# robertknight/rten

Measured on NVIDIA H100. Metric: resnet50_fp32_inferences_per_sec, higher is better.
Workload: dtype f32(tf32 mma, explicit opt-in)

## Files before the change

rten_b200/csrc/umma_gemm.cu:

```cuda
#include <cuda.h>
#include <cuda_runtime.h>

#include <algorithm>
#include <array>
#include <cmath>
#include <vector>
#include <cmath>
#include <cstdint>
#include <cstdio>
#include <cstdlib>

#include "math.cuh"
#include "ptx.cuh"
#include "rowops.h"
#include "umma_gemm.h"
#include "umma_kernel.cuh"

namespace rtb {

typedef CUresult (*EncodeTiledFn)(CUtensorMap*, CUtensorMapDataType, cuuint32_t, void*, const cuuint64_t*,
                                  const cuuint64_t*, const cuuint32_t*, const cuuint32_t*, CUtensorMapInterleave,
                                  CUtensorMapSwizzle, CUtensorMapL2promotion, CUtensorMapFloatOOBfill);

static EncodeTiledFn get_encode(rten_ctx* ctx) {
// ... 399 lines not shown
    if (!encode_map(ctx, &m.a, L.a, q.esize, L.kind == 0, q.abox, q.aes)) return RTEN_ERR_UNSUPPORTED_VALUE;
    if (!encode_map(ctx, &m.b, L.b, q.esize, L.kind == 0, bbox, bes)) return RTEN_ERR_UNSUPPORTED_VALUE;
    m.d = m.r = m.a2 = m.a_proj = m.b_proj = m.a2_proj = m.w2 = m.z = m.a;
    p.x3_cb = L.x3_cb;
    if (L.x3_cb && !encode_map(ctx, &m.a2, L.a_lo, q.esize, true, q.abox, q.aes)) return RTEN_ERR_UNSUPPORTED_VALUE;
    if (p.kb_proj) {
        p.x3_cb_proj = L.proj.x3_cb;
        if (!encode_map(ctx, &m.a_proj, L.proj.a, 4, true, q.pbox, q.pes) ||
            !encode_map(ctx, &m.b_proj, L.proj.b, 4, true, bbox, bes) ||
            (L.proj.x3_cb && !encode_map(ctx, &m.a2_proj, L.proj.a_lo, 4, true, q.pbox, q.pes)))
            return RTEN_ERR_UNSUPPORTED_VALUE;
    }
    if (p.tma_store && !encode_map(ctx, &m.d, q.od, 4, true, q.dbox, des)) {
        p.tma_store = 0;
        p.res_tma = 0;
        m.d = m.a;
    }
    if (p.res_tma && !encode_map(ctx, &m.r, q.ord, 4, true, q.dbox, des)) {
        p.res_tma = 0;
        m.r = m.a;
    }
    const Epi epi = pick_epilogue(L, p.tma_store, p.res_tma, p.splitk);
    if (epi == Epi::Generic && (L.kind == 1 || L.epi.act > 1)) p.res_tma = 0;
    if (q.chain_bytes) {
        const GemmLaunch::Chain& c = L.chain;
        const uint32_t wbox[4] = {32, (uint32_t)c.N2, 1, 1}, zbox[4] = {32, q.dbox[1], q.dbox[2], q.dbox[3]};
        if (epi != Epi::PlainF32 || (L.epi.r && !p.res_tma) || !encode_map(ctx, &m.w2, c.w, 4, true, wbox, des) ||
            !encode_map(ctx, &m.z, c.z, 4, true, zbox, des))
            return RTEN_ERR_UNSUPPORTED_VALUE;
        p.chain_n2 = c.N2;
        p.chain_passes = (L.N + p.bn - 1) / p.bn;
        p.chain_act = c.act;
        p.chain_bias = c.bias;
    }

    if (verbose)
        fprintf(stderr, "[umma_gemm] kind=%d conv=%d M=%d N=%d K=%d kb=%d kb_proj=%d tiles_m=%d bn=%d splitk=%d units=%d stages=%d tma_store=%d res_tma=%d nbuf=%d box=%dx%dx%d epi=%s%s\n",
                L.kind, L.conv, L.M, L.N, L.K, p.k_blocks, p.kb_proj, p.tiles_m, p.bn, p.splitk, p.units_total, p.stages,
                p.tma_store, p.res_tma, p.nbuf, p.tw, p.th, p.tb, epi_name(epi),
                p.chain_n2 == 64 ? " chain=64" : p.chain_n2 == 128 ? " chain=128" : "");
    if ((is_wide(p.bn) || p.kb_proj || L.epi.bias2) && !is_plain_f32(epi)) return RTEN_ERR_UNSUPPORTED_VALUE;
    const size_t smem_bytes = (size_t)p.stages * p.stage_bytes + q.chain_bytes +
                              (is_wide(p.bn) ? WIDE_SMEM_FIXED_BYTES : ps.n_stg * STG_BYTES + SMEM_FIXED_BYTES);
    using Kernel = void (*)(TmaMaps, KParams);
    static const Kernel narrow[2][7] = {
        {umma_gemm_kernel<0, Epi::Generic>, umma_gemm_kernel<0, Epi::Fast>, umma_gemm_kernel<0, Epi::FastGelu>,
         umma_gemm_kernel<0, Epi::PlainF32>, umma_gemm_kernel<0, Epi::PlainF32Gelu>, nullptr, nullptr},
        {umma_gemm_kernel<1, Epi::Generic>, umma_gemm_kernel<1, Epi::Fast>, umma_gemm_kernel<1, Epi::FastGelu>, nullptr,
         nullptr, umma_gemm_kernel<1, Epi::PlainI8>, umma_gemm_kernel<1, Epi::PlainI8Gelu>}};
    const Kernel kern = !is_wide(p.bn)              ? narrow[L.kind][(int)epi]
                        : p.chain_n2 == 64         ? umma_wide_kernel<Epi::PlainF32, 64>
                        : p.chain_n2 == 128        ? umma_wide_kernel<Epi::PlainF32, 128>
                        : epi == Epi::PlainF32Gelu ? umma_wide_kernel<Epi::PlainF32Gelu>
                                                   : umma_wide_kernel<Epi::PlainF32>;

    const int threads = is_wide(p.bn) ? WIDE_THREADS : NUM_THREADS;
    return launch(ctx, "umma_gemm launch", kern, {std::min(p.units_total, ctx->num_sms), threads, smem_bytes, 227 * 1024, true}, m, p);
}

static std::vector<long long> tune_key(const GemmLaunch& L, const Prepared& q) {
    const EpilogueDesc& e = L.epi;
    std::vector<long long> k = {L.kind, L.conv, L.M, L.N, L.K, L.z0, L.z1, q.tma_store, q.res_tma, e.act, e.bias_kind,
                                e.r != nullptr, (e.za != nullptr || e.za8 != nullptr), e.zb != nullptr, e.scale != nullptr,
                                L.a.strides[1], L.b.strides[1], L.x3_cb};
    if (L.conv) {
        const ConvGeom& g = L.g;
        for (long long v : {g.B, g.H, g.W, g.C, g.OH, g.OW, g.kh, g.kw, g.sy, g.sx, g.dy, g.dx, g.pt, g.pl}) k.push_back(v);
    }
    if (L.proj.C > 0) {
        const GemmLaunch::Projection& pr = L.proj;
        for (int64_t v : {(int64_t)-1, (int64_t)pr.C, (int64_t)pr.stride, (int64_t)pr.x3_cb, pr.a.dims[1], pr.a.dims[2],
                          pr.a.strides[1], pr.a.strides[2], pr.a.strides[3], pr.b.strides[1]})
            k.push_back(v);
    }
    return k;
}

static Plan plan_from_array(const std::array<int, 3>& a) {
    Plan pl;
    pl.bn = a[0];
    pl.splitk = a[1];
    pl.nbuf = a[2];
    return pl;
}

static rten_status launch_tf32x3(rten_ctx* ctx, const GemmLaunch& L0) {
    GemmLaunch L = L0;
    long long d0 = 0, d0p = 0;
    auto split = [&](const OperandDesc& src, OperandDesc& dst, int role, void* into) -> rten_status {
        const long long planes = role == 2 ? 1 : 3;
        long long dims[4], strides[4], n = planes * d0p;
        for (int i = 0; i < 4; i++) {
            dims[i] = (i > 0 && src.strides[i] == 0) ? 1 : src.dims[i];
            strides[i] = src.strides[i];
        }
        for (int i = 1; i < 4; i++) n *= dims[i];
        void* buf = into;
        if (!buf) RTB_TRY(temp_alloc(ctx, (size_t)n * 4, &buf));
        RTB_TRY(launch_tf32x3_split(ctx, (const float*)src.base, (float*)buf, dims, strides, d0p, role));
        dst = src;
        dst.base = buf;
        dst.dims[0] = planes * d0p;
        long long st = planes * d0p;
        for (int i = 1; i < 4; i++) {
            dst.strides[i] = (src.strides[i] == 0 && src.dims[i] > 1) ? 0 : st;
            st *= dims[i];
        }
        return RTEN_OK;
    };
    auto split_source = [&](const OperandDesc& a0, const OperandDesc& b0, void** slot, const void* a_lo_base,
                            OperandDesc& a, OperandDesc& b, OperandDesc& a_lo, int& x3_cb) -> rten_status {
        d0 = a0.dims[0];
        d0p = (d0 + 3) / 4 * 4;
        if (b0.dims[0] != d0) return RTEN_ERR_UNSUPPORTED_VALUE;
        if (slot && !getenv("RTEN_B200_X3_NO_CACHE")) {
            if (!*slot && !ctx->capturing) {
                long long n = 3 * d0p;
                for (int i = 1; i < 4; i++) n *= (b0.strides[i] == 0 ? 1 : b0.dims[i]);
                void* buf = nullptr;
                if (cudaMalloc(&buf, (size_t)n * 4) != cudaSuccess) return fail(ctx, RTEN_ERR_CUDA, "cudaMalloc failed for the 3xTF32 copy of a prepacked operand");
                OperandDesc tmp;
                const rten_status st = split(b0, tmp, 1, buf);
                if (st != RTEN_OK) {
                    cudaFree(buf);
                    return st;
                }
                *slot = buf;
            }
        }
        if (slot && *slot && !getenv("RTEN_B200_X3_NO_CACHE")) {
            b = b0;
            b.base = *slot;
            b.dims[0] = 3 * d0p;
            long long st = 3 * d0p;
            for (int i = 1; i < 4; i++) {
                const long long di = b0.strides[i] == 0 ? 1 : b0.dims[i];
                b.strides[i] = (b0.strides[i] == 0 && b0.dims[i] > 1) ? 0 : st;
                st *= di;
            }
        } else {
            RTB_TRY(split(b0, b, 1, nullptr));
        }
        const bool two_plane = d0 % 32 == 0 && tma_compatible(a0, 4, 4) && !getenv("RTEN_B200_X3_THREE_PLANES");
        if (two_plane && a_lo_base) {
            a_lo = a0;
            a_lo.base = a_lo_base;
            x3_cb = (int)(d0 / 32);
        } else if (two_plane) {
            RTB_TRY(split(a0, a_lo, 2, nullptr));
            x3_cb = (int)(d0 / 32);
        } else {
            RTB_TRY(split(a0, a, 0, nullptr));
        }
        return RTEN_OK;
    };
    RTB_TRY(split_source(L0.a, L0.b, L0.b_x3_slot, L0.a_lo_base, L.a, L.b, L.a_lo, L.x3_cb));
    if (L.conv)
        L.g.C = (int)(3 * d0p);
    L.K = L.conv ? (int)(L0.K / d0 * 3 * d0p) : (int)(3 * d0p);
    L.b_x3_slot = nullptr;
    L.a_lo_base = nullptr;
    if (L0.proj.C > 0) {
        RTB_TRY(split_source(L0.proj.a, L0.proj.b, L0.proj.b_x3_slot, nullptr, L.proj.a, L.proj.b, L.proj.a_lo, L.proj.x3_cb));
        L.proj.C = (int)(3 * d0p);
        L.proj.b_x3_slot = nullptr;
    }
    const int saved = ctx->f32_mode;
    ctx->f32_mode = RTEN_F32_TF32;
    const rten_status st = launch_umma_gemm(ctx, L);
    ctx->f32_mode = saved;
    return st;
}

rten_status launch_umma_gemm(rten_ctx* ctx, const GemmLaunch& L) {
    if (L.chain.N2 > 0) {
        if (L.kind != 0 || ctx->f32_mode != RTEN_F32_TF32 || L.x3_cb || getenv("RTEN_B200_NO_CHAIN"))
            return RTEN_ERR_UNSUPPORTED_VALUE;
        Prepared q;
        RTB_TRY(prepare_launch(ctx, L, q));
        Plan pl;
        pl.bn = 128;
        pl.nbuf = 2;
        return launch_plan(ctx, L, q, pl, getenv("RTEN_B200_VERBOSE") != nullptr);
    }
    if (L.kind == 0 && ctx->f32_mode == RTEN_F32_TF32X3) return launch_tf32x3(ctx, L);
    if (L.conv && L.kind == 0 && L.g.kh * L.g.kw > 1 && !L.x3_cb && !L.proj.C) {
        const rten_status hs = launch_umma_halo_conv(ctx, L);
        if (hs != RTEN_ERR_UNSUPPORTED_VALUE) return hs;
    }
    Prepared q;
    RTB_TRY(prepare_launch(ctx, L, q));
    const bool verbose = getenv("RTEN_B200_VERBOSE") != nullptr;
    const bool forced = getenv("RTEN_B200_FORCE_BN") || getenv("RTEN_B200_FORCE_SPLITK");
    if (!forced && !ctx->tune_cache.empty()) {
        auto hit = ctx->tune_cache.find(tune_key(L, q));
        if (hit != ctx->tune_cache.end()) {
            PlanShape ps;
            if (hit->second[0] < 0) {
                const rten_status hs = launch_umma_halo_conv(ctx, L, hit->second[1], hit->second[2]);
                if (hs != RTEN_ERR_UNSUPPORTED_VALUE) return hs;
            } else
            if (plan_shape(q, plan_from_array(hit->second), ps)) return launch_plan(ctx, L, q, plan_from_array(hit->second), verbose);
            if (verbose) fprintf(stderr, "[umma_gemm] recorded plan no longer valid for this problem: re-planning\n");
            ctx->tune_cache.erase(hit);
        }
    }
    std::vector<std::pair<double, Plan>> cands;
    enumerate_plans(q, ctx->num_sms, cands);
    if (cands.empty()) return RTEN_ERR_UNSUPPORTED_VALUE;
    Plan plan = cands[0].second;

    if (forced) {
        const char* fb = getenv("RTEN_B200_FORCE_BN");
        const char* fs = getenv("RTEN_B200_FORCE_SPLITK");
        bool found = false;
        for (const auto& c : cands) {
            const Plan& x = c.second;
            if (fb && x.bn != atoi(fb)) continue;
            if (fs && x.splitk != atoi(fs)) continue;
            plan = x;
            found = true;
            break;
        }
        if (!found) {
            ctx->forced_misses++;
            if (verbose) fprintf(stderr, "[umma_gemm] no valid plan matches the forced fields: using the model's choice\n");
            if (getenv("RTEN_B200_FORCE_STRICT"))
                return fail(ctx, RTEN_ERR_INVALID_VALUE, "no launch plan matches the forced RTEN_B200_FORCE_* fields");
        } else {
            ctx->forced_hits++;
        }
    } else if (ctx->autotune || !ctx->tune_cache.empty()) {
        const std::vector<long long> key = tune_key(L, q);
        auto it = ctx->tune_cache.find(key);
        PlanShape ps_hit;
        if (it != ctx->tune_cache.end() && it->second[0] < 0) {
            const rten_status hs = launch_umma_halo_conv(ctx, L, it->second[1], it->second[2]);
            if (hs != RTEN_ERR_UNSUPPORTED_VALUE) return hs;
            ctx->tune_cache.erase(it);
        } else if (it != ctx->tune_cache.end() && plan_shape(q, plan_from_array(it->second), ps_hit)) {
            plan = plan_from_array(it->second);
        } else if (ctx->autotune) {
            cudaStreamCaptureStatus cs = cudaStreamCaptureStatusNone;
            cudaStreamIsCapturing(ctx->stream, &cs);
            const bool safe = !ctx->capturing && cs == cudaStreamCaptureStatusNone &&
                              (L.epi.r == nullptr || (const void*)L.epi.r != (const void*)L.epi.d);
            if (safe) {
                cudaEvent_t e0, e1;
                cudaEventCreate(&e0);
                cudaEventCreate(&e1);
                const size_t ncand = std::min<size_t>(cands.size(), 24);
                size_t ws_max = 0;
                for (size_t i = 0; i < ncand; i++) {
                    PlanShape ps;
                    if (plan_shape(q, cands[i].second, ps)) ws_max = std::max(ws_max, splitk_ws_bytes(ps, cands[i].second));
                }
                void* ws = nullptr;
                if (ws_max) {
                    RTB_TRY(ensure_splitk_counters(ctx));
                    RTB_TRY(temp_alloc(ctx, ws_max, &ws));
                    cudaStreamSynchronize(ctx->stream);
                }
                double best_ms = 1e30;
                int reps = 4;
                std::vector<std::pair<double, size_t>> timed;
                auto time_plan = [&](const Plan& x, int n) -> double {
                    if (launch_plan(ctx, L, q, x, false, ws) != RTEN_OK) return -1.0;
                    cudaEventRecord(e0, ctx->stream);
                    bool ok = true;
                    for (int r = 0; r < n && ok; r++) ok = launch_plan(ctx, L, q, x, false, ws) == RTEN_OK;
                    cudaEventRecord(e1, ctx->stream);
                    if (cudaEventSynchronize(e1) != cudaSuccess || !ok) return -1.0;
                    float t = 0.f;
                    cudaEventElapsedTime(&t, e0, e1);
                    return (double)t / n;
                };
                for (size_t i = 0; i < ncand; i++) {
                    const Plan& x = cands[i].second;
                    double ms = time_plan(x, reps);
                    if (ms < 0) continue;
                    timed.emplace_back(ms, i);
                    if (verbose)
                        fprintf(stderr, "[autotune] bn=%d splitk=%d nbuf=%d model=%.0f -> %.2f us\n", x.bn, x.splitk, x.nbuf,
                                cands[i].first, ms * 1e3);
                    if (ms < best_ms) {
                        best_ms = ms;
                        plan = x;
                    }
                    reps = std::max(4, std::min(32, (int)(0.15 / std::max(best_ms, 1e-3))));
                }
                std::sort(timed.begin(), timed.end());
                best_ms = 1e30;
                for (size_t k = 0; k < std::min<size_t>(3, timed.size()); k++) {
                    const Plan& x = cands[timed[k].second].second;
                    const double again = time_plan(x, 2 * reps);
                    const double ms = again < 0 ? timed[k].first : again;
                    if (ms < best_ms) {
                        best_ms = ms;
                        plan = x;
                    }
                }
                int halo_bn = 0, halo_T = 0;
                if (L.conv && L.kind == 0 && L.g.kh * L.g.kw > 1 && !L.x3_cb && !L.proj.C && !getenv("RTEN_B200_NO_HALO")) {
                    for (int hbn : {32, 64})
                        for (int hT : {1}) {
                            if (hbn > L.N) continue;
                            auto time_halo = [&](int n) -> double {
                                if (launch_umma_halo_conv(ctx, L, hbn, hT) != RTEN_OK) return -1.0;
                                cudaEventRecord(e0, ctx->stream);
                                bool ok = true;
                                for (int r = 0; r < n && ok; r++) ok = launch_umma_halo_conv(ctx, L, hbn, hT) == RTEN_OK;
                                cudaEventRecord(e1, ctx->stream);
                                if (cudaEventSynchronize(e1) != cudaSuccess || !ok) return -1.0;
                                float t = 0.f;
                                cudaEventElapsedTime(&t, e0, e1);
                                return (double)t / n;
                            };
                            double ms = time_halo(reps);
                            if (ms > 0 && ms < best_ms * 1.05) ms = time_halo(2 * reps);
                            if (verbose && ms > 0) fprintf(stderr, "[autotune] halo bn=%d T=%d -> %.2f us\n", hbn, hT, ms * 1e3);
                            if (ms > 0 && ms < best_ms * 0.97) {
                                best_ms = ms;
                                halo_bn = hbn;
                                halo_T = hT;
                            }
                        }
                }
                cudaEventDestroy(e0);
                cudaEventDestroy(e1);
                if (halo_bn) {
                    ctx->tune_cache[key] = {-1, halo_bn, halo_T};
                    return launch_umma_halo_conv(ctx, L, halo_bn, halo_T);
                }
                ctx->tune_cache[key] = {plan.bn, plan.splitk, plan.nbuf};
            }
        }
    }
    return launch_plan(ctx, L, q, plan, verbose);
}

}
```

rten_b200/csrc/umma_halo.cu:

```cuda
#include <cuda.h>
#include <cuda_runtime.h>

#include <algorithm>
#include <cstdint>
#include <cstdio>
#include <cstdlib>
#include <cstring>

#include "math.cuh"
#include "ptx.cuh"
#include "umma_gemm.h"

namespace rtb {

namespace {

constexpr int HALO_THREADS = 416;
constexpr int HALO_PRODUCER = 12;
constexpr int HB_MAX = 8;

struct HaloParams {
    int B, OH, OW, N, C;
    int kh, kw, pt, pl;
    int P;
    int R;
    int tb;
    int nr;
    int T;
    int bn;
    int c_blocks;
    int taps;
    int strips, units_n, units_total;
    int acc_stages;
    int b_stages;
    int tps;
    uint32_t patch_bytes, patch_tx, b_bytes;
    uint32_t tap_off[32];
    uint32_t m_img, m_P;
    EpilogueDesc epi;
};

__device__ __forceinline__ void halo_unit(const HaloParams& p, int u, int& n0, int& oy0, int& b0) {
    const int nt = u % p.units_n;
    const int rest = u / p.units_n;
    const int st = rest % p.strips;
    n0 = nt * p.bn;
    oy0 = st * p.R;
    b0 = (rest / p.strips) * p.tb;
}

template <int N>
__device__ __forceinline__ void halo_mma(const HaloParams& p, uint64_t* patch_full, uint64_t* patch_empty, uint64_t* b_full,
                                         uint64_t* b_empty, uint64_t* acc_full, uint64_t* acc_empty, uint8_t* patch0,
                                         uint8_t* bring, uint32_t acc_smem) {
    const int lane = threadIdx.x & 31;
    uint32_t pphase = 0, bphase = 0, aphase = 0;
    int ps = 0, bs = 0, it = 0;
    for (int u = blockIdx.x; u < p.units_total; u += gridDim.x, it++) {
        const int acc = it & 1;
        float d0[N / 2], d1[N / 2];
#pragma unroll
        for (int i = 0; i < N / 2; i++) d0[i] = d1[i] = 0.0f;
        const int steps = p.c_blocks * p.taps;
        for (int i = 0, tap = 0; i < steps; i++) {
            if (tap == 0) mbar_wait(&patch_full[ps], (pphase >> ps) & 1);
            mbar_wait(&b_full[bs], (bphase >> bs) & 1);
            wgmma_fence();
            const uint32_t sa = smem_u32(patch0 + (size_t)ps * p.patch_bytes) + p.tap_off[tap];
            const uint64_t adesc0 = make_kmajor_sw128_desc(sa), adesc1 = make_kmajor_sw128_desc(sa + 64 * 128);
            const uint64_t bdesc = make_kmajor_sw128_desc(smem_u32(bring + (size_t)bs * p.b_bytes));
#pragma unroll
            for (int k = 0; k < 4; k++) {
                wgmma_k<0, 0, N>(d0, adesc0 + 2 * k, bdesc + 2 * k);
                wgmma_k<0, 0, N>(d1, adesc1 + 2 * k, bdesc + 2 * k);
            }
            wgmma_commit();
            wgmma_wait<0>();
            if (lane == 0) mbar_arrive(&b_empty[bs]);
            bphase ^= 1u << bs;
            if (++bs == p.b_stages) bs = 0;
            if (++tap == p.taps) {
                tap = 0;
                if (lane == 0) mbar_arrive(&patch_empty[ps]);
                pphase ^= 1u << ps;
                ps ^= 1;
            }
        }
        mbar_wait(&acc_empty[acc], ((aphase >> acc) & 1) ^ 1);
        aphase ^= 1u << acc;
        acc_store_frag<N>(acc_smem, d0, 0, acc * 64);
        acc_store_frag<N>(acc_smem, d1, 64, acc * 64);
        mbar_arrive(&acc_full[acc]);
    }
}

__global__ void __launch_bounds__(HALO_THREADS, 1)
umma_halo_kernel(const __grid_constant__ CUtensorMap tma_a, const __grid_constant__ CUtensorMap tma_b, const __grid_constant__ HaloParams p) {
    extern __shared__ uint8_t smem_raw[];
    uint8_t* base = reinterpret_cast<uint8_t*>((reinterpret_cast<uintptr_t>(smem_raw) + 1023) & ~uintptr_t(1023));
    uint64_t* patch_full = reinterpret_cast<uint64_t*>(base);
    uint64_t* patch_empty = patch_full + 2;
    uint64_t* b_full = patch_empty + 2;
    uint64_t* b_empty = b_full + HB_MAX;
    uint64_t* acc_full = b_empty + HB_MAX;
    uint64_t* acc_empty = acc_full + 2;
    float* bias_s = reinterpret_cast<float*>(base + 1024);
    const uint32_t acc_smem = smem_u32(base + 2048);
    uint8_t* stage0 = base + 2048 + ACC_SMEM_BYTES;
    uint8_t* patch0 = stage0 + 2 * 16384;
    uint8_t* bring = patch0 + 2 * (size_t)p.patch_bytes;
    const int warp = threadIdx.x >> 5, lane = threadIdx.x & 31;

    if (threadIdx.x == 0) {
        tma_prefetch_desc(&tma_a);
        tma_prefetch_desc(&tma_b);
    }
    if (warp == 1) {
        if (lane < 2) {
            mbar_init(&patch_full[lane], 1);
            mbar_init(&patch_empty[lane], 4);
            mbar_init(&acc_full[lane], 128);
            mbar_init(&acc_empty[lane], 8);
        }
        if (lane < HB_MAX) {
            mbar_init(&b_full[lane], 1);
            mbar_init(&b_empty[lane], 4);
        }
        fence_mbar_init();
    }
    __syncthreads();
    pdl_wait();
    pdl_launch_dependents();

    if (warp == HALO_PRODUCER) {
        uint32_t pphase = 0, bphase = 0;
        int ps = 0, bs = 0;
        for (int u = blockIdx.x; u < p.units_total; u += gridDim.x) {
            int n0, oy0, b0;
            halo_unit(p, u, n0, oy0, b0);
            for (int cb = 0; cb < p.c_blocks; cb++) {
                mbar_wait(&patch_empty[ps], ((pphase >> ps) & 1) ^ 1);
                if (elect_one()) {
                    mbar_expect_tx(&patch_full[ps], p.patch_tx);
                    tma_load_4d(patch0 + (size_t)ps * p.patch_bytes, &tma_a, &patch_full[ps], cb * 32, -p.pl, oy0 - p.pt, b0);
                }
                __syncwarp();
                pphase ^= 1u << ps;
                ps ^= 1;
                for (int tap = 0; tap < p.taps; tap += p.tps) {
                    mbar_wait(&b_empty[bs], ((bphase >> bs) & 1) ^ 1);
                    if (elect_one()) {
                        mbar_expect_tx(&b_full[bs], p.b_bytes);
                        tma_load_4d(bring + (size_t)bs * p.b_bytes, &tma_b, &b_full[bs], cb * 32, n0, tap, 0);
                    }
                    __syncwarp();
                    bphase ^= 1u << bs;
                    if (++bs == p.b_stages) bs = 0;
                }
            }
        }
    } else if (warp < 4) {
        if (p.bn == 32)
            halo_mma<32>(p, patch_full, patch_empty, b_full, b_empty, acc_full, acc_empty, patch0, bring, acc_smem);
        else
            halo_mma<64>(p, patch_full, patch_empty, b_full, b_empty, acc_full, acc_empty, patch0, bring, acc_smem);
    } else if (warp >= 4) {
        const EpilogueDesc& e = p.epi;
        const int q = warp & 3, grp = (warp - 4) >> 2;
        const int r = q * 32 + lane;
        const bool has_bias = e.bias_kind == 1;
        const bool do_relu = e.act == 1;
        const uint32_t img_slots = (uint32_t)(p.nr * p.P);
        uint8_t* stg = stage0 + grp * 16384;
        uint8_t* rowp = stg + r * 128;
        const int sw = r & 7;
        float* bias_g = bias_s + grp * 128;
        const int piece = lane & 7;
        uint32_t aphase = 0;
        int it = 0;
        float* outp = reinterpret_cast<float*>(e.d);
        for (int u = blockIdx.x; u < p.units_total; u += gridDim.x, it++) {
            int n0, oy0, b0;
            halo_unit(p, u, n0, oy0, b0);
            const int acc = p.acc_stages == 2 ? (it & 1) : 0;
            float bv = 0.0f;
            if (has_bias) {
                const int c = (r >> 5) * 64 + grp * 32 + (r & 31);
                if (c < p.bn && n0 + c < p.N) bv = __ldg(e.bias + n0 + c);
            }
            mbar_wait(&acc_full[acc], (aphase >> acc) & 1);
            aphase ^= 1u << acc;
            bias_g[r] = bv;
            for (int t = 0; t < p.T; t++) {
                long long off[8];
                unsigned valid = 0;
#pragma unroll
                for (int i = 0; i < 8; i++) {
                    const uint32_t slot = (uint32_t)(t * 128 + q * 32 + i * 4 + (lane >> 3));
                    const uint32_t img = __umulhi(slot, p.m_img);
                    const uint32_t rem = slot - img * img_slots;
                    const uint32_t yy = __umulhi(rem, p.m_P);
                    const uint32_t ox = rem - yy * (uint32_t)p.P;
                    const int oy = oy0 + (int)yy, b = b0 + (int)img;
                    if ((int)img < p.tb && b < p.B && (int)yy < p.R && oy < p.OH && (int)ox < p.OW) valid |= 1u << i;
                    off[i] = (long long)b * e.s_z0 + (long long)oy * e.s_row + (long long)ox * e.s_z1 + n0 + piece * 4;
                }
                const uint32_t t_row = ((uint32_t)(q * 32) << 16) + acc * 64 + t * p.bn;
                int k = 0;
                for (int c0 = grp * 32; c0 < p.bn; c0 += 64, k++) {
                    uint32_t v[32];
                    acc_ld(acc_smem, t_row + c0, v);
                    asm volatile("bar.sync %0, 128;" ::"r"(1 + grp) : "memory");
                    const float4* bq = reinterpret_cast<const float4*>(bias_g + 32 * k);
#pragma unroll
                    for (int j = 0; j < 32; j += 4) {
                        const float4 bb = bq[j >> 2];
                        add_f32x2(v[j], v[j + 1], bb.x, bb.y);
                        add_f32x2(v[j + 2], v[j + 3], bb.z, bb.w);
                        if (do_relu) {
#pragma unroll
                            for (int w = 0; w < 4; w++) v[j + w] = __float_as_uint(fmaxf(__uint_as_float(v[j + w]), 0.0f));
                        }
                    }
#pragma unroll
                    for (int j = 0; j < 8; j++)
                        *reinterpret_cast<uint4*>(rowp + ((j ^ sw) << 4)) = make_uint4(v[4 * j], v[4 * j + 1], v[4 * j + 2], v[4 * j + 3]);
                    asm volatile("bar.sync %0, 128;" ::"r"(1 + grp) : "memory");
                    if (n0 + c0 < p.N) {
#pragma unroll
                        for (int i = 0; i < 8; i++) {
                            const int sl = q * 32 + i * 4 + (lane >> 3);
                            const uint4 d = *reinterpret_cast<const uint4*>(stg + sl * 128 + ((piece ^ (sl & 7)) << 4));
                            if (valid & (1u << i)) *reinterpret_cast<uint4*>(outp + off[i] + c0) = d;
                        }
                    }
                }
            }
            __syncwarp();
            if (lane == 0) mbar_arrive(&acc_empty[acc]);
        }
    }
}

}

rten_status launch_umma_halo_conv(rten_ctx* ctx, const GemmLaunch& L, int force_bn, int force_T) {
    if (getenv("RTEN_B200_NO_HALO")) return RTEN_ERR_UNSUPPORTED_VALUE;
    if (!force_bn) {
        const char* on = getenv("RTEN_B200_HALO");
        if (!on || atoi(on) == 0) return RTEN_ERR_UNSUPPORTED_VALUE;
    }
    if (!L.conv || L.kind != 0) return RTEN_ERR_UNSUPPORTED_VALUE;
    const ConvGeom& g = L.g;
    const EpilogueDesc& e = L.epi;
    if (g.sy != 1 || g.sx != 1 || g.dy != 1 || g.dx != 1 || g.kh * g.kw < 2 || g.kh * g.kw > 32) return RTEN_ERR_UNSUPPORTED_VALUE;
    if (g.C % 32 || g.C < 32) return RTEN_ERR_UNSUPPORTED_VALUE;
    if (L.N % 32 || L.N < 32) return RTEN_ERR_UNSUPPORTED_VALUE;
    if (e.r || e.range || e.bias_kind == 2 || e.act > 1 || e.s_col != 1 || e.d_is_i32 || e.alpha != 1.0f) return RTEN_ERR_UNSUPPORTED_VALUE;
    auto al16 = [](const void* q) { return (reinterpret_cast<uintptr_t>(q) & 15) == 0; };
    if (!al16(e.d) || (e.s_z0 & 3) || (e.s_row & 3) || (e.s_z1 & 3) || (e.bias_kind == 1 && !al16(e.bias))) return RTEN_ERR_UNSUPPORTED_VALUE;
    if (!tma_compatible(L.a, 4, 4) || !tma_compatible(L.b, 4, 4)) return RTEN_ERR_UNSUPPORTED_VALUE;
    HaloParams p;
    memset(&p, 0, sizeof(p));
    p.B = g.B;
    p.OH = g.OH;
    p.OW = g.OW;
    p.N = L.N;
    p.C = g.C;
    p.kh = g.kh;
    p.kw = g.kw;
    p.pt = g.pt;
    p.pl = g.pl;
    p.P = g.OW + g.kw - 1;
    p.c_blocks = g.C / 32;
    p.taps = g.kh * g.kw;
    p.epi = e;
    if (p.P > 256) return RTEN_ERR_UNSUPPORTED_VALUE;
    const int num_sms = ctx->num_sms;
    double best = 1e30;
    int bbn = 0, bT = 0, bR = 0, btb = 0, btps = 1;
    const char* fbn = getenv("RTEN_B200_HALO_BN");
    const char* fT = getenv("RTEN_B200_HALO_T");
    const int want_bn = force_bn ? force_bn : (fbn ? atoi(fbn) : 0), want_T = force_T ? force_T : (fT ? atoi(fT) : 0);
    for (int bn = 32; bn <= std::min(L.N, 64); bn += 32) {
        if (L.N % bn) continue;
        if (want_bn && bn != want_bn) continue;
        for (int T = 1; T <= 1; T++) {
            if (want_T && T != want_T) continue;
            const int img_slots = (g.OH + g.kh - 1) * p.P;
            int tb = 1, R = 0;
            if (g.OH * p.P <= T * 128) {
                R = g.OH;
                tb = 1 + (T * 128 - g.OH * p.P) / img_slots;
                tb = std::min(tb, g.B);
            } else {
                R = (T * 128) / p.P;
                if (R < 1) continue;
            }
            const int nr = R + g.kh - 1;
            if (nr > 256 || tb > 256) continue;
            const long long alloc_slots = (long long)T * 128 + (g.kh - 1) * p.P + g.kw - 1;
            const long long loaded_slots = (long long)tb * nr * p.P;
            const long long patch_bytes = (std::max(alloc_slots, loaded_slots) * 128 + 1023) / 1024 * 1024;
            const long long budget = 227 * 1024 - 3072 - ACC_SMEM_BYTES - 2 * 16384 - 2 * patch_bytes;
            int tps = 0;
            for (int cand : {1}) {
                if ((long long)cand * bn * 128 * 3 <= budget) {
                    tps = cand;
                    break;
                }
            }
            if (!tps || tps > 256) continue;
            const long long strips = (g.OH + R - 1) / R;
            const long long units = strips * ((g.B + tb - 1) / tb) * (L.N / bn);
            const double waves = std::ceil((double)units / num_sms);
            const double mma = (double)p.c_blocks * ((double)T * p.taps * 4.0 * std::max(42.0, bn / 2.0) + 320.0 * (p.taps / tps));
            const double bytes = (double)p.c_blocks * (loaded_slots * 128.0 + (double)p.taps * bn * 128.0);
            const double ingest = bytes / 55.0;
            const double epi = (double)T * (bn / 32.0) * 350.0 / 2.0;
            const int acc_stages = 2;
            const double unit = std::max(mma, ingest) + (acc_stages == 2 ? 0.25 * epi : epi) + 800.0;
            const double cost = waves * unit + 4000.0;
            if (cost < best) {
                best = cost;
                bbn = bn;
                bT = T;
                bR = R;
                btb = tb;
                btps = tps;
            }
        }
    }
    if (!bbn) return RTEN_ERR_UNSUPPORTED_VALUE;
    p.bn = bbn;
    p.T = bT;
    p.R = bR;
    p.tb = btb;
    p.nr = p.R + g.kh - 1;
    p.acc_stages = 2;
    p.strips = (g.OH + p.R - 1) / p.R;
    p.units_n = L.N / p.bn;
    p.units_total = p.strips * ((g.B + p.tb - 1) / p.tb) * p.units_n;
    const long long alloc_slots = (long long)p.T * 128 + (g.kh - 1) * p.P + g.kw - 1;
    const long long loaded_slots = (long long)p.tb * p.nr * p.P;
    p.patch_bytes = (uint32_t)((std::max(alloc_slots, loaded_slots) * 128 + 1023) / 1024 * 1024);
    p.patch_tx = (uint32_t)(loaded_slots * 128);
    p.tps = btps;
    p.b_bytes = (uint32_t)(p.tps * p.bn) * 128u;
    p.b_stages = (int)std::min<long long>(HB_MAX, (227 * 1024 - 3072 - ACC_SMEM_BYTES - 2 * 16384 - 2LL * p.patch_bytes) / p.b_bytes);
    for (int ky = 0; ky < g.kh; ky++)
        for (int kx = 0; kx < g.kw; kx++) p.tap_off[ky * g.kw + kx] = (uint32_t)((ky * p.P + kx) * 128);
    p.m_img = (uint32_t)(0x100000000ull / (unsigned long long)(p.nr * p.P)) + 1u;
    p.m_P = (uint32_t)(0x100000000ull / (unsigned long long)p.P) + 1u;

    uint32_t abox[4] = {32u, (uint32_t)p.P, (uint32_t)p.nr, (uint32_t)p.tb}, ones[4] = {1, 1, 1, 1};
    uint32_t bbox[4] = {32u, (uint32_t)p.bn, (uint32_t)p.tps, 1u};
    CUtensorMap map_a, map_b;
    if (!encode_map(ctx, &map_a, L.a, 4, true, abox, ones)) return RTEN_ERR_UNSUPPORTED_VALUE;
    if (!encode_map(ctx, &map_b, L.b, 4, true, bbox, ones)) return RTEN_ERR_UNSUPPORTED_VALUE;
    if (getenv("RTEN_B200_VERBOSE"))
        fprintf(stderr, "[umma_halo] B=%d %dx%d C=%d N=%d k=%dx%d: bn=%d T=%d R=%d tb=%d P=%d units=%d acc_stages=%d b_stages=%d tps=%d patch=%u B\n", g.B,
                g.OH, g.OW, g.C, L.N, g.kh, g.kw, p.bn, p.T, p.R, p.tb, p.P, p.units_total, p.acc_stages, p.b_stages, p.tps, p.patch_bytes);
    const size_t smem = 1024  + 2048  + ACC_SMEM_BYTES + 2 * 16384  + 2 * (size_t)p.patch_bytes + (size_t)p.b_stages * p.b_bytes;
    return launch(ctx, "umma_halo launch", umma_halo_kernel, {std::min(p.units_total, num_sms), HALO_THREADS, smem, 227 * 1024, true},
                  map_a, map_b, p);
}

}
```

Baseline: 16810.

## Restructure halo conv kernel into two consumer warpgroups with register epilogue

Replaces the single MMA warpgroup plus separate epilogue warps (which staged accumulators through shared memory) with two consumer warpgroups that each run wgmma on half the tile and write bias/ReLU results directly from registers via a swizzled staging buffer. The producer warpgroup gives up registers via setmaxnreg so consumers get more, and wgmma_wait<1> lets buffer release overlap the next MMA. It also widens the tile search to bn=128 and T=2 and updates the cost model. The epilogue no longer overlaps the next unit's MMA, which may cost throughput on some layers.

```diff
diff --git a/rten_b200/csrc/umma_gemm.cu b/rten_b200/csrc/umma_gemm.cu
--- a/rten_b200/csrc/umma_gemm.cu
+++ b/rten_b200/csrc/umma_gemm.cu
@@ -725,9 +725,9 @@
                 }
                 int halo_bn = 0, halo_T = 0;
                 if (L.conv && L.kind == 0 && L.g.kh * L.g.kw > 1 && !L.x3_cb && !L.proj.C && !getenv("RTEN_B200_NO_HALO")) {
-                    for (int hbn : {32, 64})
-                        for (int hT : {1}) {
-                            if (hbn > L.N) continue;
+                    for (int hbn : {32, 64, 128})
+                        for (int hT : {1, 2}) {
+                            if (hbn > L.N || (hT == 1 && hbn > 64)) continue;
                             auto time_halo = [&](int n) -> double {
                                 if (launch_umma_halo_conv(ctx, L, hbn, hT) != RTEN_OK) return -1.0;
                                 cudaEventRecord(e0, ctx->stream);
diff --git a/rten_b200/csrc/umma_halo.cu b/rten_b200/csrc/umma_halo.cu
--- a/rten_b200/csrc/umma_halo.cu
+++ b/rten_b200/csrc/umma_halo.cu
@@ -15,9 +15,11 @@
 
 namespace {
 
-constexpr int HALO_THREADS = 416;
-constexpr int HALO_PRODUCER = 12;
+constexpr int HALO_THREADS = 384;
 constexpr int HB_MAX = 8;
+constexpr int HALO_STG_BYTES = 128 * 128;
+constexpr int HALO_FIXED_BYTES = 1024 + 2048 + 2 * HALO_STG_BYTES;
+constexpr int HALO_SMEM_MAX = 227 * 1024;
 
 struct HaloParams {
     int B, OH, OW, N, C;
@@ -31,9 +33,7 @@
     int c_blocks;
     int taps;
     int strips, units_n, units_total;
-    int acc_stages;
     int b_stages;
-    int tps;
     uint32_t patch_bytes, patch_tx, b_bytes;
     uint32_t tap_off[32];
     uint32_t m_img, m_P;
@@ -50,50 +50,125 @@
 }
 
 template <int N>
-__device__ __forceinline__ void halo_mma(const HaloParams& p, uint64_t* patch_full, uint64_t* patch_empty, uint64_t* b_full,
-                                         uint64_t* b_empty, uint64_t* acc_full, uint64_t* acc_empty, uint8_t* patch0,
-                                         uint8_t* bring, uint32_t acc_smem) {
-    const int lane = threadIdx.x & 31;
-    uint32_t pphase = 0, bphase = 0, aphase = 0;
-    int ps = 0, bs = 0, it = 0;
-    for (int u = blockIdx.x; u < p.units_total; u += gridDim.x, it++) {
-        const int acc = it & 1;
-        float d0[N / 2], d1[N / 2];
-#pragma unroll
-        for (int i = 0; i < N / 2; i++) d0[i] = d1[i] = 0.0f;
+__device__ __forceinline__ void halo_wgmma(float (&d)[N / 2], uint64_t adesc, uint64_t bdesc) {
+    if constexpr (N == 128) wgmma_tf32_n128(d, adesc, bdesc);
+    else wgmma_k<0, 0, N>(d, adesc, bdesc);
+}
+
+template <int N, int H>
+__device__ __forceinline__ void halo_consumer(const HaloParams& p, uint64_t* patch_full, uint64_t* patch_empty,
+                                              uint64_t* b_full, uint64_t* b_empty, const uint8_t* patch0,
+                                              const uint8_t* bring, uint8_t* stg, float* bias_s) {
+    const int w = (threadIdx.x >> 7) - 1;
+    const int t = threadIdx.x & 127;
+    const int q = t >> 5, lane = threadIdx.x & 31;
+    const int slot0 = 64 * H * w;
+    const int row0 = 16 * q + (lane >> 2);
+    const int sw = lane >> 2;
+    const int cq = lane & 3;
+    const int piece = lane & 7;
+    const EpilogueDesc& e = p.epi;
+    const bool do_relu = e.act == 1;
+    const uint32_t img_slots = (uint32_t)(p.nr * p.P);
+    const uint32_t bar_id = 1 + w;
+    float* outp = reinterpret_cast<float*>(e.d);
+    uint32_t pphase = 0, bphase = 0;
+    int ps = 0, bs = 0;
+    for (int u = blockIdx.x; u < p.units_total; u += gridDim.x) {
+        int n0, oy0, b0;
+        halo_unit(p, u, n0, oy0, b0);
+        if (t < N) bias_s[t] = (e.bias_kind == 1 && n0 + t < p.N) ? __ldg(e.bias + n0 + t) : 0.0f;
+        float d[H][N / 2];
+#pragma unroll
+        for (int h = 0; h < H; h++)
+#pragma unroll
+            for (int i = 0; i < N / 2; i++) d[h][i] = 0.0f;
         const int steps = p.c_blocks * p.taps;
+        int prev_b = -1, prev_p = -1;
         for (int i = 0, tap = 0; i < steps; i++) {
             if (tap == 0) mbar_wait(&patch_full[ps], (pphase >> ps) & 1);
             mbar_wait(&b_full[bs], (bphase >> bs) & 1);
+#pragma unroll
+            for (int h = 0; h < H; h++) wgmma_fence_operand(d[h]);
             wgmma_fence();
-            const uint32_t sa = smem_u32(patch0 + (size_t)ps * p.patch_bytes) + p.tap_off[tap];
-            const uint64_t adesc0 = make_kmajor_sw128_desc(sa), adesc1 = make_kmajor_sw128_desc(sa + 64 * 128);
+            const uint32_t sa = smem_u32(patch0 + (size_t)ps * p.patch_bytes) + p.tap_off[tap] + slot0 * 128;
             const uint64_t bdesc = make_kmajor_sw128_desc(smem_u32(bring + (size_t)bs * p.b_bytes));
 #pragma unroll
-            for (int k = 0; k < 4; k++) {
-                wgmma_k<0, 0, N>(d0, adesc0 + 2 * k, bdesc + 2 * k);
-                wgmma_k<0, 0, N>(d1, adesc1 + 2 * k, bdesc + 2 * k);
-            }
+            for (int k = 0; k < 4; k++)
+#pragma unroll
+                for (int h = 0; h < H; h++) halo_wgmma<N>(d[h], make_kmajor_sw128_desc(sa + h * 64 * 128) + 2 * k, bdesc + 2 * k);
             wgmma_commit();
-            wgmma_wait<0>();
-            if (lane == 0) mbar_arrive(&b_empty[bs]);
+#pragma unroll
+            for (int h = 0; h < H; h++) wgmma_fence_operand(d[h]);
+            wgmma_wait<1>();
+            if (lane == 0) {
+                if (prev_b >= 0) mbar_arrive(&b_empty[prev_b]);
+                if (prev_p >= 0) mbar_arrive(&patch_empty[prev_p]);
+            }
+            prev_b = bs;
+            prev_p = -1;
             bphase ^= 1u << bs;
             if (++bs == p.b_stages) bs = 0;
             if (++tap == p.taps) {
                 tap = 0;
-                if (lane == 0) mbar_arrive(&patch_empty[ps]);
+                prev_p = ps;
                 pphase ^= 1u << ps;
                 ps ^= 1;
             }
         }
-        mbar_wait(&acc_empty[acc], ((aphase >> acc) & 1) ^ 1);
-        aphase ^= 1u << acc;
-        acc_store_frag<N>(acc_smem, d0, 0, acc * 64);
-        acc_store_frag<N>(acc_smem, d1, 64, acc * 64);
-        mbar_arrive(&acc_full[acc]);
-    }
-}
-
+        wgmma_wait<0>();
+#pragma unroll
+        for (int h = 0; h < H; h++) wgmma_fence_operand(d[h]);
+        if (lane == 0) {
+            mbar_arrive(&b_empty[prev_b]);
+            mbar_arrive(&patch_empty[prev_p]);
+        }
+        long long off[4 * H];
+        unsigned valid = 0;
+#pragma unroll
+        for (int i = 0; i < 4 * H; i++) {
+            const uint32_t slot = (uint32_t)(slot0 + i * 16 + q * 4 + (lane >> 3));
+            const uint32_t img = __umulhi(slot, p.m_img);
+            const uint32_t rem = slot - img * img_slots;
+            const uint32_t yy = __umulhi(rem, p.m_P);
+            const uint32_t ox = rem - yy * (uint32_t)p.P;
+            const int oy = oy0 + (int)yy, b = b0 + (int)img;
+            if ((int)img < p.tb && b < p.B && (int)yy < p.R && oy < p.OH && (int)ox < p.OW) valid |= 1u << i;
+            off[i] = (long long)b * e.s_z0 + (long long)oy * e.s_row + (long long)ox * e.s_z1 + n0 + piece * 4;
+        }
+#pragma unroll
+        for (int k = 0; k < N / 32; k++) {
+            asm volatile("bar.sync %0, 128;" ::"r"(bar_id) : "memory");
+#pragma unroll
+            for (int h = 0; h < H; h++)
+#pragma unroll
+                for (int j = 0; j < 4; j++) {
+                    const float2 bb = *reinterpret_cast<const float2*>(bias_s + 32 * k + 8 * j + 2 * cq);
+#pragma unroll
+                    for (int r = 0; r < 2; r++) {
+                        const int i0 = 16 * k + 4 * j + 2 * r;
+                        uint32_t v0 = __float_as_uint(d[h][i0]), v1 = __float_as_uint(d[h][i0 + 1]);
+                        add_f32x2(v0, v1, bb.x, bb.y);
+                        if (do_relu) {
+                            v0 = __float_as_uint(fmaxf(__uint_as_float(v0), 0.0f));
+                            v1 = __float_as_uint(fmaxf(__uint_as_float(v1), 0.0f));
+                        }
+                        uint8_t* px = stg + (64 * h + row0 + 8 * r) * 128 + (((2 * j + (cq >> 1)) ^ sw) << 4) + 8 * (cq & 1);
+                        *reinterpret_cast<uint2*>(px) = make_uint2(v0, v1);
+                    }
+                }
+            asm volatile("bar.sync %0, 128;" ::"r"(bar_id) : "memory");
+#pragma unroll
+            for (int i = 0; i < 4 * H; i++) {
+                const int sl = i * 16 + q * 4 + (lane >> 3);
+                const uint4 v = *reinterpret_cast<const uint4*>(stg + sl * 128 + ((piece ^ (sl & 7)) << 4));
+                if (valid & (1u << i)) *reinterpret_cast<uint4*>(outp + off[i] + 32 * k) = v;
+            }
+        }
+    }
+}
+
+template <int N, int H>
 __global__ void __launch_bounds__(HALO_THREADS, 1)
 umma_halo_kernel(const __grid_constant__ CUtensorMap tma_a, const __grid_constant__ CUtensorMap tma_b, const __grid_constant__ HaloParams p) {
     extern __shared__ uint8_t smem_raw[];
@@ -102,12 +177,9 @@
     uint64_t* patch_empty = patch_full + 2;
     uint64_t* b_full = patch_empty + 2;
     uint64_t* b_empty = b_full + HB_MAX;
-    uint64_t* acc_full = b_empty + HB_MAX;
-    uint64_t* acc_empty = acc_full + 2;
     float* bias_s = reinterpret_cast<float*>(base + 1024);
-    const uint32_t acc_smem = smem_u32(base + 2048);
-    uint8_t* stage0 = base + 2048 + ACC_SMEM_BYTES;
-    uint8_t* patch0 = stage0 + 2 * 16384;
+    uint8_t* stage0 = base + 2048;
+    uint8_t* patch0 = stage0 + 2 * HALO_STG_BYTES;
     uint8_t* bring = patch0 + 2 * (size_t)p.patch_bytes;
     const int warp = threadIdx.x >> 5, lane = threadIdx.x & 31;
 
@@ -118,13 +190,11 @@
     if (warp == 1) {
         if (lane < 2) {
             mbar_init(&patch_full[lane], 1);
-            mbar_init(&patch_empty[lane], 4);
-            mbar_init(&acc_full[lane], 128);
-            mbar_init(&acc_empty[lane], 8);
+            mbar_init(&patch_empty[lane], 8);
         }
         if (lane < HB_MAX) {
             mbar_init(&b_full[lane], 1);
-            mbar_init(&b_empty[lane], 4);
+            mbar_init(&b_empty[lane], 8);
         }
         fence_mbar_init();
     }
@@ -132,7 +202,9 @@
     pdl_wait();
     pdl_launch_dependents();
 
-    if (warp == HALO_PRODUCER) {
+    if (warp < 4) {
+        asm volatile("setmaxnreg.dec.sync.aligned.u32 56;");
+        if (warp != 0) return;
         uint32_t pphase = 0, bphase = 0;
         int ps = 0, bs = 0;
         for (int u = blockIdx.x; u < p.units_total; u += gridDim.x) {
@@ -147,7 +219,7 @@
                 __syncwarp();
                 pphase ^= 1u << ps;
                 ps ^= 1;
-                for (int tap = 0; tap < p.taps; tap += p.tps) {
+                for (int tap = 0; tap < p.taps; tap++) {
                     mbar_wait(&b_empty[bs], ((bphase >> bs) & 1) ^ 1);
                     if (elect_one()) {
                         mbar_expect_tx(&b_full[bs], p.b_bytes);
@@ -159,86 +231,11 @@
                 }
             }
         }
-    } else if (warp < 4) {
-        if (p.bn == 32)
-            halo_mma<32>(p, patch_full, patch_empty, b_full, b_empty, acc_full, acc_empty, patch0, bring, acc_smem);
-        else
-            halo_mma<64>(p, patch_full, patch_empty, b_full, b_empty, acc_full, acc_empty, patch0, bring, acc_smem);
-    } else if (warp >= 4) {
-        const EpilogueDesc& e = p.epi;
-        const int q = warp & 3, grp = (warp - 4) >> 2;
-        const int r = q * 32 + lane;
-        const bool has_bias = e.bias_kind == 1;
-        const bool do_relu = e.act == 1;
-        const uint32_t img_slots = (uint32_t)(p.nr * p.P);
-        uint8_t* stg = stage0 + grp * 16384;
-        uint8_t* rowp = stg + r * 128;
-        const int sw = r & 7;
-        float* bias_g = bias_s + grp * 128;
-        const int piece = lane & 7;
-        uint32_t aphase = 0;
-        int it = 0;
-        float* outp = reinterpret_cast<float*>(e.d);
-        for (int u = blockIdx.x; u < p.units_total; u += gridDim.x, it++) {
-            int n0, oy0, b0;
-            halo_unit(p, u, n0, oy0, b0);
-            const int acc = p.acc_stages == 2 ? (it & 1) : 0;
-            float bv = 0.0f;
-            if (has_bias) {
-                const int c = (r >> 5) * 64 + grp * 32 + (r & 31);
-                if (c < p.bn && n0 + c < p.N) bv = __ldg(e.bias + n0 + c);
-            }
-            mbar_wait(&acc_full[acc], (aphase >> acc) & 1);
-            aphase ^= 1u << acc;
-            bias_g[r] = bv;
-            for (int t = 0; t < p.T; t++) {
-                long long off[8];
-                unsigned valid = 0;
-#pragma unroll
-                for (int i = 0; i < 8; i++) {
-                    const uint32_t slot = (uint32_t)(t * 128 + q * 32 + i * 4 + (lane >> 3));
-                    const uint32_t img = __umulhi(slot, p.m_img);
-                    const uint32_t rem = slot - img * img_slots;
-                    const uint32_t yy = __umulhi(rem, p.m_P);
-                    const uint32_t ox = rem - yy * (uint32_t)p.P;
-                    const int oy = oy0 + (int)yy, b = b0 + (int)img;
-                    if ((int)img < p.tb && b < p.B && (int)yy < p.R && oy < p.OH && (int)ox < p.OW) valid |= 1u << i;
-                    off[i] = (long long)b * e.s_z0 + (long long)oy * e.s_row + (long long)ox * e.s_z1 + n0 + piece * 4;
-                }
-                const uint32_t t_row = ((uint32_t)(q * 32) << 16) + acc * 64 + t * p.bn;
-                int k = 0;
-                for (int c0 = grp * 32; c0 < p.bn; c0 += 64, k++) {
-                    uint32_t v[32];
-                    acc_ld(acc_smem, t_row + c0, v);
-                    asm volatile("bar.sync %0, 128;" ::"r"(1 + grp) : "memory");
-                    const float4* bq = reinterpret_cast<const float4*>(bias_g + 32 * k);
-#pragma unroll
-                    for (int j = 0; j < 32; j += 4) {
-                        const float4 bb = bq[j >> 2];
-                        add_f32x2(v[j], v[j + 1], bb.x, bb.y);
-                        add_f32x2(v[j + 2], v[j + 3], bb.z, bb.w);
-                        if (do_relu) {
-#pragma unroll
-                            for (int w = 0; w < 4; w++) v[j + w] = __float_as_uint(fmaxf(__uint_as_float(v[j + w]), 0.0f));
-                        }
-                    }
-#pragma unroll
-                    for (int j = 0; j < 8; j++)
-                        *reinterpret_cast<uint4*>(rowp + ((j ^ sw) << 4)) = make_uint4(v[4 * j], v[4 * j + 1], v[4 * j + 2], v[4 * j + 3]);
-                    asm volatile("bar.sync %0, 128;" ::"r"(1 + grp) : "memory");
-                    if (n0 + c0 < p.N) {
-#pragma unroll
-                        for (int i = 0; i < 8; i++) {
-                            const int sl = q * 32 + i * 4 + (lane >> 3);
-                            const uint4 d = *reinterpret_cast<const uint4*>(stg + sl * 128 + ((piece ^ (sl & 7)) << 4));
-                            if (valid & (1u << i)) *reinterpret_cast<uint4*>(outp + off[i] + c0) = d;
-                        }
-                    }
-                }
-            }
-            __syncwarp();
-            if (lane == 0) mbar_arrive(&acc_empty[acc]);
-        }
+    } else {
+        asm volatile("setmaxnreg.inc.sync.aligned.u32 224;");
+        const int w = (warp >> 2) - 1;
+        halo_consumer<N, H>(p, patch_full, patch_empty, b_full, b_empty, patch0, bring, stage0 + w * HALO_STG_BYTES,
+                            bias_s + w * 128);
     }
 }
 
@@ -278,15 +275,16 @@
     if (p.P > 256) return RTEN_ERR_UNSUPPORTED_VALUE;
     const int num_sms = ctx->num_sms;
     double best = 1e30;
-    int bbn = 0, bT = 0, bR = 0, btb = 0, btps = 1;
+    int bbn = 0, bT = 0, bR = 0, btb = 0;
     const char* fbn = getenv("RTEN_B200_HALO_BN");
     const char* fT = getenv("RTEN_B200_HALO_T");
     const int want_bn = force_bn ? force_bn : (fbn ? atoi(fbn) : 0), want_T = force_T ? force_T : (fT ? atoi(fT) : 0);
-    for (int bn = 32; bn <= std::min(L.N, 64); bn += 32) {
+    for (int bn = 32; bn <= std::min(L.N, 128); bn *= 2) {
         if (L.N % bn) continue;
         if (want_bn && bn != want_bn) continue;
-        for (int T = 1; T <= 1; T++) {
+        for (int T = 1; T <= 2; T++) {
             if (want_T && T != want_T) continue;
+            if (T == 1 && bn > 64) continue;
             const int img_slots = (g.OH + g.kh - 1) * p.P;
             int tb = 1, R = 0;
             if (g.OH * p.P <= T * 128) {
@@ -302,24 +300,16 @@
             const long long alloc_slots = (long long)T * 128 + (g.kh - 1) * p.P + g.kw - 1;
             const long long loaded_slots = (long long)tb * nr * p.P;
             const long long patch_bytes = (std::max(alloc_slots, loaded_slots) * 128 + 1023) / 1024 * 1024;
-            const long long budget = 227 * 1024 - 3072 - ACC_SMEM_BYTES - 2 * 16384 - 2 * patch_bytes;
-            int tps = 0;
-            for (int cand : {1}) {
-                if ((long long)cand * bn * 128 * 3 <= budget) {
-                    tps = cand;
-                    break;
-                }
-            }
-            if (!tps || tps > 256) continue;
+            const long long budget = HALO_SMEM_MAX - HALO_FIXED_BYTES - 2 * patch_bytes;
+            if ((long long)bn * 128 * 3 > budget) continue;
             const long long strips = (g.OH + R - 1) / R;
             const long long units = strips * ((g.B + tb - 1) / tb) * (L.N / bn);
             const double waves = std::ceil((double)units / num_sms);
-            const double mma = (double)p.c_blocks * ((double)T * p.taps * 4.0 * std::max(42.0, bn / 2.0) + 320.0 * (p.taps / tps));
+            const double mma = (double)p.c_blocks * p.taps * (8.0 * T * std::max(16.0, bn / 2.0) + 60.0);
             const double bytes = (double)p.c_blocks * (loaded_slots * 128.0 + (double)p.taps * bn * 128.0);
             const double ingest = bytes / 55.0;
-            const double epi = (double)T * (bn / 32.0) * 350.0 / 2.0;
-            const int acc_stages = 2;
-            const double unit = std::max(mma, ingest) + (acc_stages == 2 ? 0.25 * epi : epi) + 800.0;
+            const double epi = (double)T * 128 * bn * 4 / 16.0;
+            const double unit = std::max(mma, ingest) + epi + 800.0;
             const double cost = waves * unit + 4000.0;
             if (cost < best) {
                 best = cost;
@@ -327,7 +317,6 @@
                 bT = T;
                 bR = R;
                 btb = tb;
-                btps = tps;
             }
         }
     }
@@ -337,7 +326,6 @@
     p.R = bR;
     p.tb = btb;
     p.nr = p.R + g.kh - 1;
-    p.acc_stages = 2;
     p.strips = (g.OH + p.R - 1) / p.R;
     p.units_n = L.N / p.bn;
     p.units_total = p.strips * ((g.B + p.tb - 1) / p.tb) * p.units_n;
@@ -345,24 +333,25 @@
     const long long loaded_slots = (long long)p.tb * p.nr * p.P;
     p.patch_bytes = (uint32_t)((std::max(alloc_slots, loaded_slots) * 128 + 1023) / 1024 * 1024);
     p.patch_tx = (uint32_t)(loaded_slots * 128);
-    p.tps = btps;
-    p.b_bytes = (uint32_t)(p.tps * p.bn) * 128u;
-    p.b_stages = (int)std::min<long long>(HB_MAX, (227 * 1024 - 3072 - ACC_SMEM_BYTES - 2 * 16384 - 2LL * p.patch_bytes) / p.b_bytes);
+    p.b_bytes = (uint32_t)p.bn * 128u;
+    p.b_stages = (int)std::min<long long>(HB_MAX, (HALO_SMEM_MAX - HALO_FIXED_BYTES - 2LL * p.patch_bytes) / p.b_bytes);
     for (int ky = 0; ky < g.kh; ky++)
         for (int kx = 0; kx < g.kw; kx++) p.tap_off[ky * g.kw + kx] = (uint32_t)((ky * p.P + kx) * 128);
     p.m_img = (uint32_t)(0x100000000ull / (unsigned long long)(p.nr * p.P)) + 1u;
     p.m_P = (uint32_t)(0x100000000ull / (unsigned long long)p.P) + 1u;
 
     uint32_t abox[4] = {32u, (uint32_t)p.P, (uint32_t)p.nr, (uint32_t)p.tb}, ones[4] = {1, 1, 1, 1};
-    uint32_t bbox[4] = {32u, (uint32_t)p.bn, (uint32_t)p.tps, 1u};
+    uint32_t bbox[4] = {32u, (uint32_t)p.bn, 1u, 1u};
     CUtensorMap map_a, map_b;
     if (!encode_map(ctx, &map_a, L.a, 4, true, abox, ones)) return RTEN_ERR_UNSUPPORTED_VALUE;
     if (!encode_map(ctx, &map_b, L.b, 4, true, bbox, ones)) return RTEN_ERR_UNSUPPORTED_VALUE;
     if (getenv("RTEN_B200_VERBOSE"))
-        fprintf(stderr, "[umma_halo] B=%d %dx%d C=%d N=%d k=%dx%d: bn=%d T=%d R=%d tb=%d P=%d units=%d acc_stages=%d b_stages=%d tps=%d patch=%u B\n", g.B,
-                g.OH, g.OW, g.C, L.N, g.kh, g.kw, p.bn, p.T, p.R, p.tb, p.P, p.units_total, p.acc_stages, p.b_stages, p.tps, p.patch_bytes);
-    const size_t smem = 1024  + 2048  + ACC_SMEM_BYTES + 2 * 16384  + 2 * (size_t)p.patch_bytes + (size_t)p.b_stages * p.b_bytes;
-    return launch(ctx, "umma_halo launch", umma_halo_kernel, {std::min(p.units_total, num_sms), HALO_THREADS, smem, 227 * 1024, true},
+        fprintf(stderr, "[umma_halo] B=%d %dx%d C=%d N=%d k=%dx%d: bn=%d T=%d R=%d tb=%d P=%d units=%d b_stages=%d patch=%u B\n", g.B,
+                g.OH, g.OW, g.C, L.N, g.kh, g.kw, p.bn, p.T, p.R, p.tb, p.P, p.units_total, p.b_stages, p.patch_bytes);
+    const size_t smem = HALO_FIXED_BYTES + 2 * (size_t)p.patch_bytes + (size_t)p.b_stages * p.b_bytes;
+    auto kern = p.T == 1 ? (p.bn == 32 ? umma_halo_kernel<32, 1> : umma_halo_kernel<64, 1>)
+                         : (p.bn == 32 ? umma_halo_kernel<32, 2> : p.bn == 64 ? umma_halo_kernel<64, 2> : umma_halo_kernel<128, 2>);
+    return launch(ctx, "umma_halo launch", kern, {std::min(p.units_total, num_sms), HALO_THREADS, smem, HALO_SMEM_MAX, true},
                   map_a, map_b, p);
 }
 
```

After: 17400 (median of 6 runs). 3.5% higher.
